# ZKI-PH-ImageAnalysis/seq2squiggle

Measured on AMD Instinct MI355X. Metric: signal samples/sec at 5 kb reads (padded [chunks x 250] samples the predict path emits), higher is better.
Workload: dtype f16x3

## Files before the change

seq2squiggle_amd/csrc/s2s_hip.hip:

```cpp
#include "s2s_device.h"
#include "s2s_device_h.h"
#include "s2s_schedule.h"
#include "s2s_generic.h"
#include "s2s_generic_h.h"
#include "s2s_train.h"
#include "../../include/s2s_hip.h"
#include "s2s_event_fixed.h"
#define S2S_DTW_KERNELS
#include "s2s_dtw.h"
#include "s2s_sdtw.h"
#include "s2s_resquiggle.h"
#include "s2s_prims.h"
#include "s2s_segment.h"
#include "s2s_eventalign.h"
#include "s2s_chunk.h"
#include "s2s_kmer_model_events.h"

#include <cctype>
#include <cstdio>
#include <cstdlib>
#include <cstring>
#include <immintrin.h>
#include <map>
#include <mutex>
#include <string>
#include <vector>

template <int NQ>
__device__ __forceinline__ void relu_tiles(f32x4 (&x)[NQ][4]) {
#pragma unroll
    for (int q = 0; q < NQ; ++q)
#pragma unroll
        for (int mt = 0; mt < 4; ++mt)
#pragma unroll
            for (int r = 0; r < 4; ++r) x[q][mt][r] = relu1(x[q][mt][r]);
}

__device__ __forceinline__ int base_code(unsigned char ch) {
    return ch == 'A' ? 1 : ch == 'C' ? 2 : ch == 'G' ? 3 : ch == 'T' ? 4 : ch == '_' ? 0 : -1;
}

struct FrontChunk {
    const uint8_t* bp;
    int nv;
    unsigned long long chunk;
    const float* inj_g;
    const float* inj_zdw;
    float* slot;
    int* out_dur;
    long long dbg_idx;
    bool live;
};
#define S2S_SLOT_FLOATS S2S_PF_FLOATS

template <int NQ, bool EVAL = false>
__device__ __forceinline__ void front_embed(const ModelDev& M, const float* __restrict__ W, const FrontChunk (&io)[NQ], const int lane,
                                            f32x4 (&X)[NQ][4]) {
    const int g = lane >> 4, c = lane & 15;
    f32x4 eb[4];
#pragma unroll
    for (int ft = 0; ft < 4; ++ft) eb[ft] = ldg4(W + M.emb_b + 16 * ft + 4 * g);
#pragma unroll
    for (int q = 0; q < NQ; ++q)
#pragma unroll
        for (int ft = 0; ft < 4; ++ft) X[q][ft] = eb[ft];
    for (int j = 0; j < M.k; ++j) {
#pragma unroll
        for (int q = 0; q < NQ; ++q) {
            const int code = EVAL ? base_code(io[q].bp[c * M.k + j])
                                  : (c < io[q].nv) ? base_code(io[q].bp[c + j]) : 0;
            const float* row = W + M.emb_wt + (5 * j + (code < 0 ? 0 : code)) * 64 + 4 * g;
#pragma unroll
            for (int ft = 0; ft < 4; ++ft) {
                const f32x4 w = ldg4(row + 16 * ft);
                if (code >= 0) X[q][ft] += w;
            }
        }
    }
    relu_tiles<NQ>(X);
}

template <int NQ>
__device__ __forceinline__ void head_out(const float* __restrict__ W, const MlpOff m, f32x4 (&hid)[NQ][4], const int lane, float (&out)[NQ]) {
    const int g = lane >> 4;
    relu_tiles<NQ>(hid);
    f32x4 w[4];
#pragma unroll
    for (int mt = 0; mt < 4; ++mt) w[mt] = ldg4(W + m.w3 + 16 * mt + 4 * g);
    const float b3 = W[m.b3];
#pragma unroll
    for (int q = 0; q < NQ; ++q) {
        float part = 0.0f;
#pragma unroll
        for (int mt = 0; mt < 4; ++mt)
#pragma unroll
            for (int r = 0; r < 4; ++r) part += hid[q][mt][r] * w[mt][r];
        out[q] = softplus_t(sum_g(part) + b3);
    }
}

template <int NQ, bool EVAL = false>
__device__ __forceinline__ void front_dwell(const FrontChunk (&io)[NQ], const ParamsDev& P, const float (&sig)[NQ], const float (&cq)[NQ],
                                            const float (&rq)[NQ], const DebugDev& dbg, const int lane) {
    const int g = lane >> 4, c = lane & 15;
    float sigma = sig[0], conc = cq[0], rate = rq[0];
    FrontChunk me = io[0];
#pragma unroll
    for (int q = 1; q < NQ; ++q)
        if (g == q) { sigma = sig[q]; conc = cq[q]; rate = rq[q]; me = io[q]; }
    const bool mine = g < NQ && me.live;
    if (mine) {
        me.slot[1024 + c] = sigma;
        if (dbg.sigma) dbg.sigma[me.dbg_idx * 16 + c] = sigma;
    }
    if constexpr (EVAL) {
        if (mine) {
            dbg.conc[me.dbg_idx * 16 + c] = fmaxf(conc, 1e-8f);
            dbg.rate[me.dbg_idx * 16 + c] = fmaxf(rate, 1e-8f);
            reinterpret_cast<int*>(me.slot + 1040)[c] = me.out_dur[c];
        }
        return;
    }
    float gv;
    if (P.duration_sampling) {
        conc = fmaxf(conc, 1e-8f);
        rate = fmaxf(rate, 1e-8f);
        if (mine) {
            if (dbg.conc) dbg.conc[me.dbg_idx * 16 + c] = conc;
            if (dbg.rate) dbg.rate[me.dbg_idx * 16 + c] = rate;
        }
        if (me.inj_g) {
            gv = mine ? me.inj_g[c] : 1.0f;
        } else {
            float sg = 0.0f;
            if (mine) sg = standard_gamma(conc, (unsigned)me.chunk, (unsigned)(me.chunk >> 32), c, P.seed_lo, P.seed_hi);
            gv = fmaxf(sg / rate, 1.17549435e-38f);
        }
        gv = fmaxf(gv, 1.0f);
        gv = fmaxf(gv, P.min_duration);
    } else if (P.dwell_std <= 0.0f) {
        gv = P.dwell_mean;
    } else {
        float z;
        if (me.inj_zdw) {
            z = mine ? me.inj_zdw[c] : 0.0f;
        } else {
            const u32x4 r = philox4x32_10((unsigned)me.chunk, (unsigned)(me.chunk >> 32), c | (S2S_KIND_DWELL << 16), 0,
                                          P.seed_lo, P.seed_hi);
            z = box_muller(r.x, r.y);
        }
        gv = fmaxf(mul_then_add(z, P.dwell_std, P.dwell_mean), P.min_duration);
    }
    if (mine) {
        const float rd = fminf(fmaxf(rintf(gv), -1.0e9f), 1.0e9f);
        reinterpret_cast<int*>(me.slot + 1040)[c] = (int)rd;
        store_stream(me.out_dur + c, (int)rd);
        if (dbg.g) dbg.g[me.dbg_idx * 16 + c] = gv;
    }
}

template <int NQ>
__device__ __forceinline__ void front_emb_in(const FrontChunk (&io)[NQ], const DebugDev& dbg, f32x4 (&X)[NQ][4], const int lane) {
    if (!dbg.emb_in) return;
    const int g = lane >> 4, c = lane & 15;
#pragma unroll
    for (int q = 0; q < NQ; ++q)
#pragma unroll
        for (int ft = 0; ft < 4; ++ft) X[q][ft] = ldg4(dbg.emb_in + (io[q].dbg_idx * 16 + c) * 64 + 16 * ft + 4 * g);
}

template <int NQ>
__device__ __forceinline__ void front_store(const FrontChunk (&io)[NQ], const DebugDev& dbg, const f32x4 (&X)[NQ][4], const int lane,
                                            const bool enc) {
    const int g = lane >> 4, c = lane & 15;
    float* const dbg_dst = enc ? dbg.enc_out : dbg.emb_out;
#pragma unroll
    for (int q = 0; q < NQ; ++q) {
        if (!io[q].live) continue;
        if (enc) {
#pragma unroll
            for (int ft = 0; ft < 4; ++ft) *reinterpret_cast<f32x4*>(io[q].slot + c * 64 + 16 * ft + 4 * g) = X[q][ft];
        }
        if (dbg_dst) {
#pragma unroll
            for (int ft = 0; ft < 4; ++ft)
                *reinterpret_cast<f32x4*>(dbg_dst + (io[q].dbg_idx * 16 + c) * 64 + 16 * ft + 4 * g) = X[q][ft];
        }
    }
}

struct FrontLdsF32 { static constexpr int BYTES = AttnLds<1>::BYTES; };
template <bool EVAL = false>
__device__ __forceinline__ void frontend_f32(const ModelDev& M, const float* __restrict__ W, const FrontChunk (&io)[1],
                                             const ParamsDev& P, char* __restrict__ lds_raw, const DebugDev& dbg, const int lane) {
    const int g = lane >> 4, c = lane & 15;
    f32x4 X[1][4];
    front_embed<1, EVAL>(M, W, io, lane, X);
#pragma unroll 1
    for (int i = 0; i < M.pre_layers; ++i) {
        f32x4 Y[1][4];
#pragma unroll
        for (int mt = 0; mt < 4; ++mt) Y[0][mt] = ldg4(W + M.pre_b[i] + 16 * mt + 4 * g);
        gemm_acc<1, 4, 4>(W + M.pre_w[i], lane, Y, X);
        relu_tiles<1>(Y);
#pragma unroll
        for (int mt = 0; mt < 4; ++mt) X[0][mt] = Y[0][mt];
    }
    front_emb_in<1>(io, dbg, X, lane);
    front_store<1>(io, dbg, X, lane, false);
    float sig[1], cq[1] = {1.0f}, rq[1] = {1.0f};
    auto head = [&](const MlpOff m, float (&out)[1]) {
        f32x4 hid[1][4];
#pragma unroll
        for (int mt = 0; mt < 4; ++mt) hid[0][mt] = ldg4(W + m.b0 + 16 * mt + 4 * g);
        gemm_acc<1, 4, 4>(W + m.w0, lane, hid, X);
        head_out<1>(W, m, hid, lane, out);
    };
    head(M.noise, sig);
    if (P.duration_sampling) { head(M.conc, cq); head(M.rate, rq); }
    front_dwell<1, EVAL>(io, P, sig, cq, rq, dbg, lane);
#pragma unroll
    for (int ft = 0; ft < 4; ++ft) X[0][ft] += ldg4(W + M.pe_enc + c * 64 + 16 * ft + 4 * g);
#pragma unroll 1
    for (int l = 0; l < M.enc_layers; ++l) fft_block<1, 1, 16>(W, M.enc[l], X, reinterpret_cast<float*>(lds_raw), 0, lane);
    front_store<1>(io, dbg, X, lane, true);
}

template <int NQ, bool EVAL = false>
__device__ __forceinline__ void frontend_h16(const ModelDev& M, const float* __restrict__ W, const FrontChunk (&io)[NQ],
                                             const ParamsDev& P, const DebugDev& dbg, const int lane, const float one) {
    const int g = lane >> 4, c = lane & 15;
    DIAG_DECL;
#define FDIAG(slot) DIAG_STAMP(32 + (slot))
    f32x4 X[NQ][4];
    front_embed<NQ, EVAL>(M, W, io, lane, X);
    FDIAG(0);
#pragma unroll 1
    for (int i = 0; i < M.pre_layers; ++i) {
        HL xb[NQ][2];
        f32x4 Y[NQ][4];
#pragma unroll
        for (int q = 0; q < NQ; ++q) { xb[q][0] = split8(X[q][0], X[q][1], one); xb[q][1] = split8(X[q][2], X[q][3], one); }
        linear64_h<NQ>(W + M.pre_wh[i], W + M.pre_b[i], lane, xb, Y);
        relu_tiles<NQ>(Y);
#pragma unroll
        for (int q = 0; q < NQ; ++q)
#pragma unroll
            for (int mt = 0; mt < 4; ++mt) X[q][mt] = Y[q][mt];
    }
    front_emb_in<NQ>(io, dbg, X, lane);
    front_store<NQ>(io, dbg, X, lane, false);
    FDIAG(1);
    {
        HL Sb[NQ][2];
#pragma unroll
        for (int q = 0; q < NQ; ++q) { Sb[q][0] = split8(X[q][0], X[q][1], one); Sb[q][1] = split8(X[q][2], X[q][3], one); }
        float sig[NQ], cq[NQ], rq[NQ];
#pragma unroll
        for (int q = 0; q < NQ; ++q) { cq[q] = 1.0f; rq[q] = 1.0f; }
        auto head = [&](const MlpOff m, float (&out)[NQ]) {
            f32x4 hid[NQ][4];
            linear64_h<NQ>(W + m.w0h, W + m.b0, lane, Sb, hid);
            head_out<NQ>(W, m, hid, lane, out);
        };
        head(M.noise, sig);
        if (P.duration_sampling) { head(M.conc, cq); head(M.rate, rq); }
        FDIAG(4);
        front_dwell<NQ, EVAL>(io, P, sig, cq, rq, dbg, lane);
    }
#pragma unroll
    for (int ft = 0; ft < 4; ++ft) {
        const f32x4 pe = ldg4(W + M.pe_enc + c * 64 + 16 * ft + 4 * g);
#pragma unroll
        for (int q = 0; q < NQ; ++q) X[q][ft] += pe;
    }
    FDIAG(5);
#pragma unroll 1
    for (int l = 0; l < M.enc_layers; ++l) {
        const LayerOff L = M.enc[l];
        const float* const wl = W + L.stream_h;
        f32x4 acc[NQ][4];
        HL x1b[NQ][2];
        enc_attention_h<NQ>(W, L, wl, X, acc, lane, one);
        FDIAG(2);
        enc_ffn_begin_h<NQ>(W, L, acc, X, x1b, lane, one);
        enc_ffn_half_h<NQ>(W, L, wl + 16 * 1024, 0, x1b, X, lane, one);
        enc_ffn_half_h<NQ>(W, L, wl + 32 * 1024, 2, x1b, X, lane, one);
        layer_norm64<NQ, true>(X, W + L.ln2g, W + L.ln2b, g);
        FDIAG(3);
    }
    front_store<NQ>(io, dbg, X, lane, true);
}

#define DEC_WAVES 8
#define DEC_NQ 2
#define DEC_WPS (DEC_WAVES / 4)
#define DEC_NKT 16
static constexpr int DEC_LDS_F32 = AttnLds<DEC_NKT>::BYTES;
static constexpr int DEC_LDS_H = AttnLdsH<DEC_NQ, DEC_WAVES, DEC_NKT>::BYTES;


struct GatherRaw {
    f32x4 e[DEC_NQ][4], pe[DEC_NQ][4];
    float sg[DEC_NQ];
    int idx[DEC_NQ];
};
__device__ __forceinline__ void dec_gather_issue(const ModelDev& M, const float* __restrict__ W, const float* __restrict__ slot,
                                                 const int wave, const int lane, GatherRaw& R) {
    const int g = lane >> 4, c = lane & 15;
    const int qt0 = DEC_NQ * wave;
    int cum[16];
    {
        const int dv = reinterpret_cast<const int*>(slot + 1040)[c];
        int run = 0;
#pragma unroll
        for (int j = 0; j < 16; ++j) {
            const int dj = __builtin_amdgcn_readlane(dv, j);
            run += dj < S2S_T_DEC + 1 ? dj : S2S_T_DEC + 1;
            cum[j] = run;
        }
    }
#pragma unroll
    for (int q = 0; q < DEC_NQ; ++q) {
        const int t = 16 * (qt0 + q) + c;
        int idx = 0;
#pragma unroll
        for (int j = 0; j < 16; ++j) idx += (cum[j] <= t) ? 1 : 0;
        R.idx[q] = idx;
        const int row = idx < 16 ? idx : 0;
        const float* er = slot + row * 64 + 4 * g;
        const float* pr = W + M.pe_dec + (t < S2S_T_DEC ? t : 0) * 64 + 4 * g;
#pragma unroll
        for (int ft = 0; ft < 4; ++ft) { R.e[q][ft] = ldg4(er + 16 * ft); R.pe[q][ft] = ldg4(pr + 16 * ft); }
        R.sg[q] = slot[1024 + row];
    }
}
__device__ __forceinline__ void dec_gather_finish(const GatherRaw& R, const int wave, const int lane, f32x4 (&X)[DEC_NQ][4],
                                                  float (&sig_ext)[DEC_NQ]) {
    const int c = lane & 15;
#pragma unroll
    for (int q = 0; q < DEC_NQ; ++q) {
        const int t = 16 * (DEC_NQ * wave + q) + c;
        const bool live = R.idx[q] < 16, real = t < S2S_T_DEC;
#pragma unroll
        for (int ft = 0; ft < 4; ++ft)
            X[q][ft] = real ? ((live ? R.e[q][ft] : f32x4{0, 0, 0, 0}) + R.pe[q][ft]) : f32x4{0, 0, 0, 0};
        sig_ext[q] = live ? R.sg[q] : 0.0f;
    }
}

__device__ __forceinline__ void dec_override(const float* __restrict__ dec_in, const long long dbg_idx, const int wave, const int lane,
                                             f32x4 (&X)[DEC_NQ][4]) {
    const int g = lane >> 4, c = lane & 15;
#pragma unroll
    for (int q = 0; q < DEC_NQ; ++q) {
        const int t = 16 * (DEC_NQ * wave + q) + c;
#pragma unroll
        for (int ft = 0; ft < 4; ++ft)
            X[q][ft] = t < S2S_T_DEC ? ldg4(dec_in + (dbg_idx * S2S_T_DEC + t) * 64 + 16 * ft + 4 * g) : f32x4{0, 0, 0, 0};
    }
}

template <int MODE, bool EXACT = false>
__device__ __forceinline__ void dec_blocks(const ModelDev& M, const float* __restrict__ W, f32x4 (&X)[DEC_NQ][4],
                                           char* __restrict__ lds_raw, const int wave, const int lane, const float one,
                                           unsigned long long* diag, const float* __restrict__ next_slot = nullptr) {
    const int qt0 = DEC_NQ * wave;
#pragma unroll 1
    for (int l = 0; l < M.dec_layers; ++l) {
        float* const slot_lds = reinterpret_cast<float*>(lds_raw + DEC_LDS_H), *const sv_lds = slot_lds + S2S_SLOT_FLOATS;
        if (MODE == 1) fft_block_h<DEC_NQ, DEC_WAVES, DEC_NKT, S2S_T_DEC, true, EXACT>(W, M.dec[l], X, lds_raw, qt0, wave, lane, one, diag,
                                                                          l == M.dec_layers - 1 ? next_slot : nullptr, slot_lds, sv_lds);
        else if (MODE == 3) fft_block_h<DEC_NQ, DEC_WAVES, DEC_NKT, S2S_T_DEC, false, EXACT>(W, M.dec[l], X, lds_raw, qt0, wave, lane, one, diag,
                                                                                      nullptr, slot_lds, sv_lds);
        else           fft_block<DEC_NQ, DEC_NKT, S2S_T_DEC>(W, M.dec[l], X, reinterpret_cast<float*>(lds_raw), qt0, lane, diag);
    }
}

__device__ __forceinline__ void dec_project(const ModelDev& M, const float* __restrict__ W, const f32x4 (&X)[DEC_NQ][4],
                                            const float (&sig_ext)[DEC_NQ], const int lane, float& ys, float& se) {
    const int g = lane >> 4;
    f32x4 wo[4];
#pragma unroll
    for (int ft = 0; ft < 4; ++ft) wo[ft] = ldg4(W + M.out_w + 16 * ft + 4 * g);
    const float bo = W[M.out_b];
    ys = 0.0f; se = 0.0f;
#pragma unroll
    for (int q = 0; q < DEC_NQ; ++q) {
        float part = 0.0f;
#pragma unroll
        for (int ft = 0; ft < 4; ++ft)
#pragma unroll
            for (int r = 0; r < 4; ++r) part += X[q][ft][r] * wo[ft][r];
        const float v = relu1(sum_g(part) + bo);
        if (g == q) { ys = v; se = sig_ext[q]; }
    }
}

__device__ __forceinline__ void dec_emit(const ModelDev& M, const float ys, const float se, const unsigned long long chunk,
                                         const ParamsDev& P, const float* __restrict__ inj_z01, float* __restrict__ out_signal,
                                         const DebugDev& dbg, const long long dbg_idx, const int wave, const int lane) {
    const int g = lane >> 4, c = lane & 15;
    const int t = 16 * (DEC_NQ * wave + g) + c;
    float y = __fmul_rn(ys, M.scale);
    if (g < DEC_NQ && t < S2S_T_DEC) {
        if (dbg.y_scaled) dbg.y_scaled[dbg_idx * S2S_T_DEC + t] = ys;
        if (P.noise_std > 0.0f) {
            float z;
            if (inj_z01) {
                z = inj_z01[t];
            } else {
                const u32x4 r = philox4x32_10((unsigned)chunk, (unsigned)(chunk >> 32),
                                              (unsigned)t | (S2S_KIND_NOISE << 16), 0, P.seed_lo, P.seed_hi);
                z = box_muller(r.x, r.y);
            }
            if (dbg.z01) dbg.z01[dbg_idx * S2S_T_DEC + t] = z;
            const float sd = P.noise_sampling
                                 ? __fmul_rn(__fmul_rn(fmaxf(se, P.min_noise), P.noise_std), M.scale)
                                 : P.noise_std;
            if (y != 0.0f) y = mul_then_add(z, sd, y);
        }
        store_stream(out_signal + t, fmaxf(y, 0.0f));
    }
}

template <int MODE> struct Fused {
    static constexpr int FMODE = (MODE == 3) ? 1 : MODE;
    static constexpr int FNQ = (FMODE == 1) ? 2 : 1;
    static constexpr int GROUP = DEC_WAVES * FNQ;
    static constexpr bool PF = (MODE == 1);
    static constexpr int LDS = (MODE == 0) ? DEC_LDS_F32 : DEC_LDS_H + (S2S_SLOT_FLOATS + S2S_SV_FLOATS + S2S_PROG_INTS + S2S_Z2_FLOATS) * 4;
    static_assert(LDS + S2S_STATIC_LDS_BYTES + 16 <= 160 * 1024, "LDS per workgroup: dynamic + the static arrays in front of it");
    static_assert(FMODE == 1 || DEC_WAVES * FrontLdsF32::BYTES <= LDS, "the f32 frontend waves' K/V images share the decoder's LDS");
};
#define S2S_MAX_GROUP (2 * DEC_WAVES)
template <int MODE, bool TEST, bool EXACT = false>
__global__ __launch_bounds__(DEC_WAVES * 64, DEC_WPS) void s2s_fused_kernel(
    const ModelDev M, const float* __restrict__ W, const uint8_t* __restrict__ bases,
    const long long* __restrict__ chunk_start, const uint8_t* __restrict__ n_valid, int n_chunks, long long first_chunk,
    ParamsDev P, const float* __restrict__ inj_g_, const float* __restrict__ inj_zdw_, const float* __restrict__ inj_z01_,
    float* __restrict__ handoff, int* __restrict__ out_dur, float* __restrict__ out_signal, DebugDev dbg_, long long dbg_base,
    unsigned* __restrict__ sched) {
    using F = Fused<MODE>;
    const float* const inj_g = TEST ? inj_g_ : nullptr;
    const float* const inj_zdw = TEST ? inj_zdw_ : nullptr;
    const float* const inj_z01 = TEST ? inj_z01_ : nullptr;
    DebugDev dbg = dbg_;
    if (!TEST) { dbg = DebugDev{}; dbg.diag = dbg_.diag; dbg.stats = dbg_.stats; }
    extern __shared__ __attribute__((aligned(16))) char lds_raw[];
    const int wave = __builtin_amdgcn_readfirstlane(threadIdx.x >> 6);
    const int lane = threadIdx.x & 63;
    const int nb = S2S_T_ENC + M.k - 1;
    if constexpr (MODE != 0) att32_consts<AttnLdsH<DEC_NQ, DEC_WAVES, DEC_NKT>>(lds_raw, threadIdx.x, DEC_WAVES * 64);
    if constexpr (MODE != 0) {
        if (threadIdx.x < S2S_PROG_INTS + S2S_Z2_FLOATS)
            reinterpret_cast<int*>(lds_raw + DEC_LDS_H + (S2S_SLOT_FLOATS + S2S_SV_FLOATS) * 4)[threadIdx.x] = 0;
    }
    if (threadIdx.x == 0) {
        const unsigned long long c0 = __builtin_readcyclecounter(), r0 = __builtin_amdgcn_s_memrealtime();
        s2s_stats_lds[0] = 0;
        s2s_stats_lds[4] = (unsigned)c0; s2s_stats_lds[5] = (unsigned)(c0 >> 32);
        s2s_stats_lds[6] = (unsigned)r0; s2s_stats_lds[7] = (unsigned)(r0 >> 32);
    }
#ifdef S2S_TILEHIST
    for (int i = threadIdx.x; i < 2 * 2 * 64; i += DEC_WAVES * 64) s2s_hist_lds[i] = 0;
#endif
#ifdef S2S_DIAG
    for (int i = threadIdx.x; i < 8 * S2S_DIAG_SLOTS; i += DEC_WAVES * 64) s2s_diag_lds[i] = 0;
    const unsigned long long diag_c0 = __builtin_readcyclecounter(), diag_r0 = __builtin_amdgcn_s_memrealtime();
    __syncthreads();
#endif
    float* const slot0 = handoff + (size_t)blockIdx.x * S2S_MAX_GROUP * S2S_SLOT_FLOATS;
    auto put_group = [&](const int start, const int count) {
        s2s_stats_lds[S2S_LDS_G0] = (unsigned)start; s2s_stats_lds[S2S_LDS_N] = (unsigned)count;
    };
    auto sched_of = [&]() {
        return reinterpret_cast<unsigned*>(((unsigned long long)s2s_stats_lds[S2S_LDS_SCHED + 1] << 32) | s2s_stats_lds[S2S_LDS_SCHED]);
    };
    auto put_claim = [&](unsigned* const q, const unsigned c) {
        int start, count;
        const unsigned G = s2s_stats_lds[S2S_LDS_GRID];
        s2s_claim_range((int)s2s_stats_lds[S2S_LDS_END], (int)G, F::GROUP, (int)c, &start, &count);
        put_group(start, count);
        if (count == 0) {
            __threadfence();
            if (atomicInc(q + 1, G - 1) == G - 1) atomicExch(q, 0u);
        }
    };
    if (threadIdx.x == 0) {
        s2s_stats_lds[S2S_LDS_SCHED] = (unsigned)(unsigned long long)sched;
        s2s_stats_lds[S2S_LDS_SCHED + 1] = (unsigned)((unsigned long long)sched >> 32);
        s2s_stats_lds[S2S_LDS_GRID] = gridDim.x;
        if (sched) {
            s2s_stats_lds[S2S_LDS_END] = (unsigned)n_chunks;
            put_claim(sched, atomicAdd(sched, 1u));
        } else {
            const int lo = (int)((long long)blockIdx.x * n_chunks / gridDim.x), hi = (int)((long long)(blockIdx.x + 1) * n_chunks / gridDim.x);
            s2s_stats_lds[S2S_LDS_END] = (unsigned)hi;
            put_group(lo, hi - lo < F::GROUP ? hi - lo : F::GROUP);
        }
    }
#pragma unroll 1
    for (;;) {
        float one = 1.0f;
        asm volatile("" : "+s"(one));
        DIAG_DECL;
        __syncthreads();
        const int g0 = __builtin_amdgcn_readfirstlane((int)s2s_stats_lds[S2S_LDS_G0]);
        const int n_here = __builtin_amdgcn_readfirstlane((int)s2s_stats_lds[S2S_LDS_N]);
        if (n_here <= 0) break;
        {
            int lnf = lane;
            asm volatile("" : "+v"(lnf));
            auto chunk_of = [&](const int j, const int j_filler) {
                const bool live = j < n_here;
                const int b = g0 + (live ? j : j_filler);
                return FrontChunk{chunk_start ? bases + chunk_start[b] : bases + (size_t)b * nb, n_valid[b],
                                  (unsigned long long)(first_chunk + b), inj_g ? inj_g + (size_t)b * 16 : nullptr,
                                  inj_zdw ? inj_zdw + (size_t)b * 16 : nullptr, slot0 + j * S2S_SLOT_FLOATS,
                                  out_dur + (size_t)b * 16, dbg_base + b, live};
            };
            if constexpr (F::FMODE == 1) {
                if (n_here > DEC_WAVES) {
                    const FrontChunk io[2] = {chunk_of(2 * wave, 2 * wave), chunk_of(2 * wave + 1, 2 * wave)};
                    if (2 * wave < n_here) frontend_h16<2>(M, W, io, P, dbg, lnf, one);
                } else {
                    const FrontChunk io[1] = {chunk_of(wave, 0)};
                    if (wave < n_here) frontend_h16<1>(M, W, io, P, dbg, lnf, one);
                }
            } else {
                const FrontChunk io[1] = {chunk_of(wave, 0)};
                if (wave < n_here) frontend_f32(M, W, io, P, lds_raw + wave * FrontLdsF32::BYTES, dbg, lnf);
            }
        }
        __syncthreads();
        DIAG_STAMP(7);
        if (threadIdx.x == 0) {
            if (unsigned* const q = sched_of()) {
                put_claim(q, atomicAdd(q, 1u));
            } else {
                const int hi = (int)s2s_stats_lds[S2S_LDS_END], nx = g0 + F::GROUP;
                put_group(nx, nx >= hi ? 0 : hi - nx < F::GROUP ? hi - nx : F::GROUP);
            }
        }
        f32x4 X[DEC_NQ][4];
        float sig_ext[DEC_NQ];
        {
            int lg = lane;
            asm volatile("" : "+v"(lg));
            GatherRaw R;
            dec_gather_issue(M, W, slot0, wave, lg, R);
            dec_gather_finish(R, wave, lg, X, sig_ext);
            if (TEST && dbg.dec_in) dec_override(dbg.dec_in, dbg_base + g0, wave, lg, X);
        }
        DIAG_STAMP(8);
#pragma unroll 1
        for (int j = 0; j < ((S2S_ABL & 65536) ? 0 : n_here); ++j) {
            const int b = g0 + j;
            const float* next = slot0 + (j + 1 < n_here ? j + 1 : j) * S2S_SLOT_FLOATS;
            dec_blocks<MODE, EXACT>(M, W, X, lds_raw, wave, lane, one, dbg.diag, F::PF ? next : nullptr);
            DIAG_STAMP(15);
            int ln = lane;
            asm volatile("" : "+v"(ln));
            float ys, se;
            dec_project(M, W, X, sig_ext, ln, ys, se);
            GatherRaw R;
            if constexpr (F::PF) dec_gather_issue(M, W, reinterpret_cast<const float*>(lds_raw + DEC_LDS_H), wave, ln, R);
            else                 dec_gather_issue(M, W, next, wave, ln, R);
            dec_emit(M, ys, se, (unsigned long long)(first_chunk + b), P, inj_z01 ? inj_z01 + (size_t)b * S2S_T_DEC : nullptr,
                     out_signal + (size_t)b * S2S_T_DEC, dbg, dbg_base + b, wave, ln);
            dec_gather_finish(R, wave, ln, X, sig_ext);
            if (TEST && dbg.dec_in) dec_override(dbg.dec_in, dbg_base + g0 + (j + 1 < n_here ? j + 1 : j), wave, ln, X);
            DIAG_STAMP(9);
        }
    }
#ifdef S2S_DIAG
    DIAG_COUNT(16, __builtin_readcyclecounter() - diag_c0);
    DIAG_COUNT(17, __builtin_amdgcn_s_memrealtime() - diag_r0);
    DIAG_COUNT(18, 1ull);
    __syncthreads();
    if (dbg.diag)
        for (int i = threadIdx.x; i < 8 * S2S_DIAG_SLOTS; i += DEC_WAVES * 64)
            if (s2s_diag_lds[i]) atomicAdd(dbg.diag + i, s2s_diag_lds[i]);
#endif
    __syncthreads();
#ifdef S2S_TILEHIST
    if (dbg.diag)
        for (int i = threadIdx.x; i < 2 * 2 * 64; i += DEC_WAVES * 64)
            if (s2s_hist_lds[i]) atomicAdd(dbg.diag + i, (unsigned long long)s2s_hist_lds[i]);
#endif
    if (threadIdx.x == 0 && dbg.stats) {
        const unsigned long long c0 = ((unsigned long long)s2s_stats_lds[5] << 32) | s2s_stats_lds[4];
        const unsigned long long r0 = ((unsigned long long)s2s_stats_lds[7] << 32) | s2s_stats_lds[6];
        if (s2s_stats_lds[0]) atomicAdd(dbg.stats + S2S_STAT_REDO, (unsigned long long)s2s_stats_lds[0]);
        atomicAdd(dbg.stats + S2S_STAT_CYCLES, __builtin_readcyclecounter() - c0);
        const unsigned long long span = __builtin_amdgcn_s_memrealtime() - r0;
        atomicAdd(dbg.stats + S2S_STAT_TICKS, span);
        atomicAdd(dbg.stats + S2S_STAT_WGS, 1ull);
        atomicMax(dbg.stats + S2S_STAT_SPAN_MAX, span);
        atomicMax(dbg.stats + S2S_STAT_SPAN_MIN_INV, ~span);
    }
}

template <int MODE, bool EXACT>
__global__ __launch_bounds__(DEC_WAVES * 64, DEC_WPS) void s2s_eval_kernel(
    const ModelDev M, const float* __restrict__ W, const uint8_t* __restrict__ kmers, const int* __restrict__ dwell, int n_chunks,
    ParamsDev P, float* __restrict__ handoff, float* __restrict__ y, DebugDev dbg_) {
    using F = Fused<MODE>;
    extern __shared__ __attribute__((aligned(16))) char lds_raw[];
    const int wave = __builtin_amdgcn_readfirstlane(threadIdx.x >> 6);
    const int lane = threadIdx.x & 63;
    if constexpr (MODE != 0) att32_consts<AttnLdsH<DEC_NQ, DEC_WAVES, DEC_NKT>>(lds_raw, threadIdx.x, DEC_WAVES * 64);
    if constexpr (MODE != 0) {
        if (threadIdx.x < S2S_PROG_INTS + S2S_Z2_FLOATS)
            reinterpret_cast<int*>(lds_raw + DEC_LDS_H + (S2S_SLOT_FLOATS + S2S_SV_FLOATS) * 4)[threadIdx.x] = 0;
    }
    if (threadIdx.x == 0) s2s_stats_lds[0] = 0;
    DebugDev dbg{};
    dbg.sigma = dbg_.sigma; dbg.conc = dbg_.conc; dbg.rate = dbg_.rate;
    float* const slot0 = handoff + (size_t)blockIdx.x * S2S_MAX_GROUP * S2S_SLOT_FLOATS;
    const int lo = (int)((long long)blockIdx.x * n_chunks / gridDim.x), hi = (int)((long long)(blockIdx.x + 1) * n_chunks / gridDim.x);
    const int kb = S2S_T_ENC * M.k;
#pragma unroll 1
    for (int g0 = lo; g0 < hi; g0 += F::GROUP) {
        const int n_here = hi - g0 < F::GROUP ? hi - g0 : F::GROUP;
        float one = 1.0f;
        asm volatile("" : "+s"(one));
        __syncthreads();
        {
            int lnf = lane;
            asm volatile("" : "+v"(lnf));
            auto chunk_of = [&](const int j, const int j_filler) {
                const bool live = j < n_here;
                const int b = g0 + (live ? j : j_filler);
                return FrontChunk{kmers + (size_t)b * kb, S2S_T_ENC, (unsigned long long)b, nullptr, nullptr, slot0 + j * S2S_SLOT_FLOATS,
                                  const_cast<int*>(dwell) + (size_t)b * S2S_T_ENC, (long long)b, live};
            };
            if constexpr (F::FMODE == 1) {
                if (n_here > DEC_WAVES) {
                    const FrontChunk io[2] = {chunk_of(2 * wave, 2 * wave), chunk_of(2 * wave + 1, 2 * wave)};
                    if (2 * wave < n_here) frontend_h16<2, true>(M, W, io, P, dbg, lnf, one);
                } else {
                    const FrontChunk io[1] = {chunk_of(wave, 0)};
                    if (wave < n_here) frontend_h16<1, true>(M, W, io, P, dbg, lnf, one);
                }
            } else {
                const FrontChunk io[1] = {chunk_of(wave, 0)};
                if (wave < n_here) frontend_f32<true>(M, W, io, P, lds_raw + wave * FrontLdsF32::BYTES, dbg, lnf);
            }
        }
        __syncthreads();
        f32x4 X[DEC_NQ][4];
        float sig_ext[DEC_NQ];
        {
            int lg = lane;
            asm volatile("" : "+v"(lg));
            GatherRaw R;
            dec_gather_issue(M, W, slot0, wave, lg, R);
            dec_gather_finish(R, wave, lg, X, sig_ext);
        }
#pragma unroll 1
        for (int j = 0; j < n_here; ++j) {
            const int b = g0 + j;
            const float* next = slot0 + (j + 1 < n_here ? j + 1 : j) * S2S_SLOT_FLOATS;
            dec_blocks<MODE, EXACT>(M, W, X, lds_raw, wave, lane, one, nullptr, F::PF ? next : nullptr);
            int ln = lane;
            asm volatile("" : "+v"(ln));
            float ys, se;
            dec_project(M, W, X, sig_ext, ln, ys, se);
            GatherRaw R;
            if constexpr (F::PF) dec_gather_issue(M, W, reinterpret_cast<const float*>(lds_raw + DEC_LDS_H), wave, ln, R);
            else                 dec_gather_issue(M, W, next, wave, ln, R);
            {
                const int g = ln >> 4, t = 16 * (DEC_NQ * wave + g) + (ln & 15);
                if (g < DEC_NQ && t < S2S_T_DEC) store_stream(y + (size_t)b * S2S_T_DEC + t, ys);
            }
            dec_gather_finish(R, wave, ln, X, sig_ext);
        }
    }
}

__global__ __launch_bounds__(256) void s2s_eval_loss_kernel(const float* __restrict__ y, const float* __restrict__ target,
                                                            const float* __restrict__ sigma, const float* __restrict__ stdev,
                                                            const float* __restrict__ conc, const float* __restrict__ rate,
                                                            const int* __restrict__ dwell, int B, int te, int ts, float* __restrict__ out_loss) {
    const long long b = (long long)blockIdx.x * 4 + (threadIdx.x >> 6);
    const int lane = threadIdx.x & 63;
    if (b >= B) return;
    float se = 0.0f;
    for (int t = lane; t < ts; t += 64) {
        const float e = y[b * ts + t] - target[b * ts + t];
        se += e * e;
    }
    float nll = 0.0f, ne = 0.0f;
    if (lane < te) {
        const long long i = b * te + lane;
        const int dv = dwell[i];
        const float x = dv == 0 ? 1.0f : (float)(dv < 0 ? -dv : dv);
        const double a = conc[i], r = rate[i];
        const double am1 = a - 1.0;
        const double lp = a * log(r) + (am1 == 0.0 ? 0.0 : am1 * log((double)x)) - r * (double)x - lgamma(a);
        nll = (float)-lp;
        const float e = stdev[i] - sigma[i];
        ne = e * e;
    }
    se = gen_wave_sum(se);
    nll = gen_wave_sum(nll);
    ne = gen_wave_sum(ne);
    if (lane == 0) { out_loss[b * 3 + 0] = se; out_loss[b * 3 + 1] = nll; out_loss[b * 3 + 2] = ne; }
}

template <int TD>
__global__ __launch_bounds__(256) void s2s_count_kernel(const float* __restrict__ signal, int B, int* __restrict__ counts, int ts) {
    const int T = TD ? TD : ts;
    const int b = blockIdx.x * 4 + (threadIdx.x >> 6), lane = threadIdx.x & 63;
    if (b >= B) return;
    int n = 0;
    for (int t = lane; t < T; t += 64) n += signal[(size_t)b * T + t] != 0.0f;
#pragma unroll
    for (int o = 32; o > 0; o >>= 1) n += __shfl_xor(n, o, 64);
    if (lane == 0) counts[b] = n;
}


__global__ __launch_bounds__(256) void s2s_read_offsets_kernel(const long long* __restrict__ offs, const int* __restrict__ read_first,
                                                               int R, long long* __restrict__ out_offsets) {
    const int r = blockIdx.x * 256 + threadIdx.x;
    if (r <= R) out_offsets[r] = offs[read_first[r]];
}

__device__ __forceinline__ short s2s_dac_of(float v, float dig, float range, float offset) {
    const float raw = rintf(__fsub_rn(__fdiv_rn(__fmul_rn(v, dig), range), offset));
    return (short)(int)fminf(fmaxf(raw, -2147483648.0f), 2147483520.0f);
}

template <int TD>
__global__ __launch_bounds__(256) void s2s_compact_kernel(const float* __restrict__ signal, int B, const long long* __restrict__ offs,
                                                          const int* __restrict__ read_first, int R, float* __restrict__ out_pa,
                                                          short* __restrict__ out_dac, long long capacity, float dig, float range,
                                                          float offset, int rna, int ts) {
    const int T = TD ? TD : ts;
    const int b = blockIdx.x * 4 + (threadIdx.x >> 6), lane = threadIdx.x & 63;
    if (b >= B) return;
    long long pos = offs[b];
    long long r_lo = 0, r_hi = 0;
    if (rna && out_dac) {
        int lo = 0, hi = R;
        while (hi - lo > 1) { const int mid = (lo + hi) >> 1; if (read_first[mid] <= b) lo = mid; else hi = mid; }
        r_lo = offs[read_first[lo]];
        r_hi = offs[read_first[lo + 1]];
    }
    for (int t0 = 0; t0 < T; t0 += 64) {
        const int t = t0 + lane;
        const float v = (t < T) ? signal[(size_t)b * T + t] : 0.0f;
        const bool keep = v != 0.0f;
        const unsigned long long mask = __ballot(keep);
        const long long dst = pos + __popcll(mask & ((1ull << lane) - 1ull));
        if (keep) {
            if (out_pa && dst < capacity) out_pa[dst] = v;
            if (out_dac) {
                const long long at = rna ? (r_lo + (r_hi - 1 - dst)) : dst;
                if (at < capacity) out_dac[at] = s2s_dac_of(v, dig, range, offset);
            }
        }
        pos += __popcll(mask);
    }
}

template <int TD>
__global__ __launch_bounds__(256) void s2s_align_kernel(const float* __restrict__ signal, const int* __restrict__ dur, int B,
                                                        unsigned short* __restrict__ out_seg, int te, int ts) {
    const int T = TD ? TD : ts;
    const int b = blockIdx.x * 4 + (threadIdx.x >> 6), lane = threadIdx.x & 63;
    if (b >= B) return;
    int c = 0;
    if (lane < te) {
        const int d = dur[(size_t)b * te + lane];
        c = d < 0 ? 0 : (d > T ? T : d);
    }
#pragma unroll
    for (int o = 1; o < 64; o <<= 1) { const int y = __shfl_up(c, o, 64); if (lane >= o) c += y; }
    c = c > T ? T : c;
    int below = 0, total = 0;
    for (int t0 = 0; t0 < T; t0 += 64) {
        const int t = t0 + lane;
        const float v = (t < T) ? signal[(size_t)b * T + t] : 0.0f;
        const unsigned long long mask = __ballot(v != 0.0f);
        const int k = c - t0;
        const unsigned long long low = k >= 64 ? ~0ull : (k <= 0 ? 0ull : ((1ull << k) - 1ull));
        below += __popcll(mask & low);
        total += __popcll(mask);
    }
    const int before = __shfl_up(below, 1, 64);
    const int last = __shfl(below, te - 1, 64);
    unsigned short* row = out_seg + (size_t)b * (te + 1);
    if (lane < te) row[lane] = (unsigned short)(below - (lane ? before : 0));
    if (lane == 0) row[te] = (unsigned short)(total - last);
}

template <int TD>
__device__ __forceinline__ void s2s_slot_stats_wave(const float* __restrict__ signal, const int* __restrict__ dur, int b, int lane,
                                                    float dig, float range, float offset, int te, int ts, int& n, int& S, long long& Q,
                                                    int& n_tail, int& s_tail, long long& q_tail) {
    const int T = TD ? TD : ts;
    int c = 0;
    if (lane < te) {
        const int d = dur[(size_t)b * te + lane];
        c = d < 0 ? 0 : (d > T ? T : d);
    }
#pragma unroll
    for (int o = 1; o < 64; o <<= 1) { const int y = __shfl_up(c, o, 64); if (lane >= o) c += y; }
    c = c > T ? T : c;
    int below = 0, total = 0;
    int s_below = 0, s_total = 0;
    long long q_below = 0, q_total = 0;
    for (int t0 = 0; t0 < T; t0 += 64) {
        const int t = t0 + lane;
        const float v = (t < T) ? signal[(size_t)b * T + t] : 0.0f;
        const bool keep = v != 0.0f;
        const unsigned long long mask = __ballot(keep);
        const int q = keep ? (int)s2s_dac_of(v, dig, range, offset) : 0;
        int s = q;
        long long qq = (long long)(q * q);
#pragma unroll
        for (int o = 1; o < 64; o <<= 1) {
            const int ys = __shfl_up(s, o, 64);
            const long long yq = __shfl_up(qq, o, 64);
            if (lane >= o) { s += ys; qq += yq; }
        }
        const int k = c - t0;
        const int src = k >= 64 ? 63 : (k <= 0 ? 0 : k - 1);
        const int ps = __shfl(s, src, 64);
        const long long pq = __shfl(qq, src, 64);
        const unsigned long long low = k >= 64 ? ~0ull : (k <= 0 ? 0ull : ((1ull << k) - 1ull));
        below += __popcll(mask & low);
        total += __popcll(mask);
        if (k > 0) { s_below += ps; q_below += pq; }
        s_total += __shfl(s, 63, 64);
        q_total += __shfl(qq, 63, 64);
    }
    const int before = __shfl_up(below, 1, 64), last = __shfl(below, te - 1, 64);
    const int s_before = __shfl_up(s_below, 1, 64), s_last = __shfl(s_below, te - 1, 64);
    const long long q_before = __shfl_up(q_below, 1, 64), q_last = __shfl(q_below, te - 1, 64);
    n = below - (lane ? before : 0);
    S = s_below - (lane ? s_before : 0);
    Q = q_below - (lane ? q_before : 0);
    n_tail = total - last;
    s_tail = s_total - s_last;
    q_tail = q_total - q_last;
}

template <int TD>
__global__ __launch_bounds__(256) void s2s_event_stats_kernel(const float* __restrict__ signal, const int* __restrict__ dur, int B,
                                                              float dig, float range, float offset,
                                                              unsigned short* __restrict__ out_seg, int* __restrict__ out_sum,
                                                              long long* __restrict__ out_sumsq, int te, int ts) {
    const int b = blockIdx.x * 4 + (threadIdx.x >> 6), lane = threadIdx.x & 63;
    if (b >= B) return;
    int n, S, n_tail, s_tail;
    long long Q, q_tail;
    s2s_slot_stats_wave<TD>(signal, dur, b, lane, dig, range, offset, te, ts, n, S, Q, n_tail, s_tail, q_tail);
    const size_t row = (size_t)b * (te + 1);
    if (lane < te) {
        out_seg[row + lane] = (unsigned short)n;
        out_sum[row + lane] = S;
        out_sumsq[row + lane] = Q;
    }
    if (lane == 0) {
        out_seg[row + te] = (unsigned short)n_tail;
        out_sum[row + te] = s_tail;
        out_sumsq[row + te] = q_tail;
    }
}

#define S2S_KMER_TABLE_LDS_MAX_K 5
template <int TD, bool LDS>
__global__ __launch_bounds__(256) void s2s_kmer_table_kernel(const float* __restrict__ signal, const int* __restrict__ dur,
                                                             const unsigned char* __restrict__ read_bytes,
                                                             const long long* __restrict__ chunk_start,
                                                             const unsigned char* __restrict__ n_valid, int B, float dig, float range,
                                                             float offset, unsigned long long* __restrict__ table, int te, int ts, int k) {
    extern __shared__ unsigned long long s2s_kmer_lds[];
    const int lane = threadIdx.x & 63, rows = (1 << (2 * k)) + 1;
    if (LDS) {
        for (int i = threadIdx.x; i < rows * S2S_KMER_TABLE_FIELDS; i += 256) s2s_kmer_lds[i] = 0ull;
        __syncthreads();
    }
    for (int b0 = blockIdx.x * 4; b0 < B; b0 += gridDim.x * 4) {
        const int b = b0 + (threadIdx.x >> 6);
        if (b >= B) continue;
        int n, S, n_tail, s_tail;
        long long Q, q_tail;
        s2s_slot_stats_wave<TD>(signal, dur, b, lane, dig, range, offset, te, ts, n, S, Q, n_tail, s_tail, q_tail);
        int nv = n_valid[b];
        nv = nv > te ? te : nv;
        const bool real = lane < nv;
        int code = 0;
        if (real) {
            const unsigned char* p = read_bytes + chunk_start[b] + lane;
            bool other = false;
            for (int i = 0; i < k; ++i) {
                const unsigned char ch = p[i];
                const int d = ch == 'A' ? 0 : ch == 'C' ? 1 : ch == 'G' ? 2 : ch == 'T' ? 3 : -1;
                other |= d < 0;
                code = code * 4 + (d & 3);
            }
            if (other) code = rows - 1;
        }
        int occ = real ? 1 : 0, ev = (real && n > 0) ? 1 : 0;
        if (!ev) { n = 0; S = 0; Q = 0; }
        long long nn = (long long)n * n;
        bool issue = real;
        unsigned long long todo = __ballot(real);
        while (todo) {
            const int first = __ffsll((long long)todo) - 1;
            const int lc = __shfl(code, first, 64);
            const bool mine = real && code == lc;
            const unsigned long long same = __ballot(mine);
            todo &= ~same;
            if (__popcll(same) < 2) continue;
            int r_ev = mine ? ev : 0, r_n = mine ? n : 0, r_s = mine ? S : 0;
            long long r_nn = mine ? nn : 0, r_q = mine ? Q : 0;
#pragma unroll
            for (int o = 32; o > 0; o >>= 1) {
                r_ev += __shfl_xor(r_ev, o, 64);
                r_n += __shfl_xor(r_n, o, 64);
                r_s += __shfl_xor(r_s, o, 64);
                r_nn += __shfl_xor(r_nn, o, 64);
                r_q += __shfl_xor(r_q, o, 64);
            }
            if (lane == first) { occ = __popcll(same); ev = r_ev; n = r_n; S = r_s; nn = r_nn; Q = r_q; }
            else if (mine) issue = false;
        }
        if (issue) {
            const unsigned long long f[S2S_KMER_TABLE_FIELDS] = {(unsigned long long)occ, (unsigned long long)ev, (unsigned long long)(long long)n,
                                                                 (unsigned long long)nn, (unsigned long long)(long long)S,
                                                                 (unsigned long long)Q};
            const int fields = ev ? S2S_KMER_TABLE_FIELDS : 1;
            if (LDS) {
// ... 1545 lines not shown
```

Baseline: 760.6 million.

## Pack base codes via cross-lane permutes and double-buffer embedding row loads

Each lane now reads its bases once (one byte per lane in the non-eval path) and builds 4-bit packed k-mer codes for every position through ds_bpermute. This replaces the k dependent byte loads per position. The embedding accumulation loop becomes a software-pipelined loop that issues the weight-row loads for the next pair of positions before adding the current pair, so memory latency overlaps with arithmetic. The cost is more live registers for the two weight buffers, extra cross-lane permute traffic, and a hard cap of k at 16.

```diff
diff --git a/seq2squiggle_amd/csrc/s2s_hip.hip b/seq2squiggle_amd/csrc/s2s_hip.hip
--- a/seq2squiggle_amd/csrc/s2s_hip.hip
+++ b/seq2squiggle_amd/csrc/s2s_hip.hip
@@ -36,8 +36,14 @@
             for (int r = 0; r < 4; ++r) x[q][mt][r] = relu1(x[q][mt][r]);
 }
 
-__device__ __forceinline__ int base_code(unsigned char ch) {
-    return ch == 'A' ? 1 : ch == 'C' ? 2 : ch == 'G' ? 3 : ch == 'T' ? 4 : ch == '_' ? 0 : -1;
+__device__ __forceinline__ unsigned base_nibble(unsigned char ch) {
+    unsigned n = ch == '_' ? 1u : 0u;
+    n = ch == 'A' ? 2u : n;
+    n = ch == 'C' ? 3u : n;
+    n = ch == 'G' ? 4u : n;
+    n = ch == 'T' ? 5u : n;
+    asm volatile("" : "+v"(n));
+    return n;
 }
 
 struct FrontChunk {
@@ -50,13 +56,70 @@
     int* out_dur;
     long long dbg_idx;
     bool live;
+    bool whole;
 };
 #define S2S_SLOT_FLOATS S2S_PF_FLOATS
+
+#define S2S_MAX_K 16
+#define EMB_BW 2
+
+template <int NQ, bool EVAL>
+__device__ __forceinline__ void front_letters(const FrontChunk (&io)[NQ], const int lane, const int k, unsigned (&codes)[NQ][S2S_MAX_K / 8]) {
+    const int c = lane & 15;
+#pragma unroll
+    for (int q = 0; q < NQ; ++q)
+#pragma unroll
+        for (int h = 0; h < S2S_MAX_K / 8; ++h) codes[q][h] = 0;
+    if constexpr (EVAL) {
+        const int g = lane >> 4;
+        unsigned char raw[NQ][S2S_MAX_K / 4];
+#pragma unroll
+        for (int q = 0; q < NQ; ++q)
+#pragma unroll
+            for (int i = 0; i < S2S_MAX_K / 4; ++i) raw[q][i] = io[q].bp[(unsigned)(c * k + (g + 4 * i < k ? g + 4 * i : k - 1))];
+#pragma unroll
+        for (int q = 0; q < NQ; ++q) {
+#pragma unroll
+            for (int i = 0; i < S2S_MAX_K / 4; ++i) codes[q][i >> 1] |= base_nibble(raw[q][i]) << (4 * (g + 4 * (i & 1)));
+#pragma unroll
+            for (int h = 0; h < S2S_MAX_K / 8; ++h) {
+                codes[q][h] |= (unsigned)__builtin_amdgcn_ds_bpermute(4 * (lane ^ 16), (int)codes[q][h]);
+                codes[q][h] |= (unsigned)__builtin_amdgcn_ds_bpermute(4 * (lane ^ 32), (int)codes[q][h]);
+            }
+        }
+    } else {
+        const int l = lane & 31, mine = NQ == 2 ? lane >> 5 : 0;
+        const uint8_t* bp = io[0].bp;
+        int nv = io[0].nv;
+        if (NQ == 2 && mine) { bp = io[NQ - 1].bp; nv = io[NQ - 1].nv; }
+        unsigned char ch = '_';
+        if (io[0].whole ? l < S2S_T_ENC + k - 1 : l < nv + k - 1) ch = bp[l];
+        const int nib = (int)base_nibble(ch);
+#pragma unroll
+        for (int q = 0; q < NQ; ++q) {
+#pragma unroll
+            for (int j = 0; j < S2S_MAX_K; ++j)
+                codes[q][j >> 3] |= (unsigned)__builtin_amdgcn_ds_bpermute(4 * (32 * q + c + j), nib) << (4 * (j & 7));
+        }
+    }
+    const unsigned m0 = k < 8 ? (1u << (4 * k)) - 1 : ~0u;
+    const unsigned m1 = k <= 8 ? 0u : k < 16 ? (1u << (4 * (k - 8))) - 1 : ~0u;
+#pragma unroll
+    for (int q = 0; q < NQ; ++q) {
+        const bool pad = !EVAL && c >= io[q].nv;
+        codes[q][0] = (pad ? 0x11111111u : codes[q][0]) & m0;
+        codes[q][1] = (pad ? 0x11111111u : codes[q][1]) & m1;
+    }
+}
 
 template <int NQ, bool EVAL = false>
 __device__ __forceinline__ void front_embed(const ModelDev& M, const float* __restrict__ W, const FrontChunk (&io)[NQ], const int lane,
                                             f32x4 (&X)[NQ][4]) {
-    const int g = lane >> 4, c = lane & 15;
+    const int g = lane >> 4;
+    int k = M.k;
+    asm volatile("" : "+s"(k));
+    unsigned codes[NQ][S2S_MAX_K / 8];
+    front_letters<NQ, EVAL>(io, lane, k, codes);
     f32x4 eb[4];
 #pragma unroll
     for (int ft = 0; ft < 4; ++ft) eb[ft] = ldg4(W + M.emb_b + 16 * ft + 4 * g);
@@ -64,18 +127,47 @@
     for (int q = 0; q < NQ; ++q)
 #pragma unroll
         for (int ft = 0; ft < 4; ++ft) X[q][ft] = eb[ft];
-    for (int j = 0; j < M.k; ++j) {
-#pragma unroll
-        for (int q = 0; q < NQ; ++q) {
-            const int code = EVAL ? base_code(io[q].bp[c * M.k + j])
-                                  : (c < io[q].nv) ? base_code(io[q].bp[c + j]) : 0;
-            const float* row = W + M.emb_wt + (5 * j + (code < 0 ? 0 : code)) * 64 + 4 * g;
-#pragma unroll
-            for (int ft = 0; ft < 4; ++ft) {
-                const f32x4 w = ldg4(row + 16 * ft);
-                if (code >= 0) X[q][ft] += w;
+    auto code_of = [&](const int q, const int j) {
+        return (int)(((j < 8 ? codes[q][0] : codes[q][1]) >> (4 * (j & 7))) & 15) - 1;
+    };
+    auto issue = [&](const int j0, f32x4 (&w)[EMB_BW][NQ][4]) {
+#pragma unroll
+        for (int b = 0; b < EMB_BW; ++b) {
+            const int j = j0 + b < k ? j0 + b : k - 1;
+#pragma unroll
+            for (int q = 0; q < NQ; ++q) {
+                const int code = code_of(q, j);
+                const float* row = W + M.emb_wt + (5 * j + (code < 0 ? 0 : code)) * 64 + 4 * g;
+#pragma unroll
+                for (int ft = 0; ft < 4; ++ft) w[b][q][ft] = ldg4(row + 16 * ft);
             }
         }
+    };
+    auto add = [&](const int j0, const f32x4 (&w)[EMB_BW][NQ][4]) {
+#pragma unroll
+        for (int b = 0; b < EMB_BW; ++b) {
+            const int j = j0 + b < S2S_MAX_K ? j0 + b : S2S_MAX_K - 1;
+            const bool in = j0 + b < k;
+#pragma unroll
+            for (int q = 0; q < NQ; ++q) {
+                asm volatile("" : : "v"(w[b][q][3]));
+                const bool known = in && code_of(q, j) >= 0;
+#pragma unroll
+                for (int ft = 0; ft < 4; ++ft)
+                    if (known) X[q][ft] += w[b][q][ft];
+            }
+        }
+    };
+    f32x4 wa[EMB_BW][NQ][4], wb[EMB_BW][NQ][4];
+    issue(0, wa);
+#pragma unroll 1
+    for (int j0 = 0;; j0 += 2 * EMB_BW) {
+        if (j0 + EMB_BW < k) issue(j0 + EMB_BW, wb);
+        add(j0, wa);
+        if (j0 + EMB_BW >= k) break;
+        if (j0 + 2 * EMB_BW < k) issue(j0 + 2 * EMB_BW, wa);
+        add(j0 + EMB_BW, wb);
+        if (j0 + 2 * EMB_BW >= k) break;
     }
     relu_tiles<NQ>(X);
 }
@@ -518,7 +610,7 @@
                 return FrontChunk{chunk_start ? bases + chunk_start[b] : bases + (size_t)b * nb, n_valid[b],
                                   (unsigned long long)(first_chunk + b), inj_g ? inj_g + (size_t)b * 16 : nullptr,
                                   inj_zdw ? inj_zdw + (size_t)b * 16 : nullptr, slot0 + j * S2S_SLOT_FLOATS,
-                                  out_dur + (size_t)b * 16, dbg_base + b, live};
+                                  out_dur + (size_t)b * 16, dbg_base + b, live, chunk_start == nullptr};
             };
             if constexpr (F::FMODE == 1) {
                 if (n_here > DEC_WAVES) {
@@ -634,7 +726,7 @@
                 const bool live = j < n_here;
                 const int b = g0 + (live ? j : j_filler);
                 return FrontChunk{kmers + (size_t)b * kb, S2S_T_ENC, (unsigned long long)b, nullptr, nullptr, slot0 + j * S2S_SLOT_FLOATS,
-                                  const_cast<int*>(dwell) + (size_t)b * S2S_T_ENC, (long long)b, live};
+                                  const_cast<int*>(dwell) + (size_t)b * S2S_T_ENC, (long long)b, live, true};
             };
             if constexpr (F::FMODE == 1) {
                 if (n_here > DEC_WAVES) {
```

New measurement: 760.9 million (median of 5 runs). Within noise of the previous version (+0.0%).
